# jean-pierreBoth/kmerutils

Measured on AMD Instinct MI355X. Metric: Gbases/sec k-mer+sketch throughput, k=31, 200 sketches/read, higher is better.
Workload: dtype u64; 1 GPU; ont_k31: 746333 ONT-shaped reads (log-normal lengths, 8% errors), 4.38e+09 bases, k=31, ProbMinHash3a m=200 + kmercount 8-bit; workload_name=ont_k31, reads_per_gpu=746333, bases_per_gpu=4379626696, kmers_per_gpu=4357236706, k=31, sketch_size=200, sketch=True, count=True, parallelism=reads sharded x1

## Files before the change

### kmerutils_amd/csrc/kmu_device.h

```cpp
#pragma once

#include <hip/hip_runtime.h>
#include <stdint.h>

#include "../../include/kmu.h"

#define KMU_WAVE 64

namespace kmu {

__device__ __forceinline__ uint32_t code2b(uint32_t c) {
    uint32_t x = (c >> 1) & 3u;
    return x ^ (x >> 1);
}
__device__ __forceinline__ bool is_acgt(uint32_t c) {
    uint32_t u = c & 0xDFu;
    return (u == 'A') | (u == 'C') | (u == 'G') | (u == 'T');
}
__device__ __forceinline__ uint32_t codes4_ascii(uint32_t c) {
    uint32_t x = (c >> 1) & 0x03030303u;
    x ^= (x >> 1) & 0x01010101u;
    return (x * 0x40100401u) >> 24;
}
__device__ __forceinline__ uint32_t diff4_ascii(uint32_t c) {
    const uint32_t u = c & 0xDFDFDFDFu;
    const uint32_t t = (u >> 2) & ~(u >> 1) & 0x01010101u;
    const uint32_t e = 0x40404040u | (u & 0x06060606u) | (t << 4) | (t ^ 0x01010101u);
    return u ^ e;
}
__device__ __forceinline__ uint32_t nonzero4(uint32_t d) {
    const uint32_t nz = (((d & 0x7F7F7F7Fu) + 0x7F7F7F7Fu) | d) & 0x80808080u;
    return (((nz >> 7) * 0x01020408u) >> 24) & 0xFu;
}
__device__ __forceinline__ uint32_t pack16_ascii(uint4 v, uint32_t &bad) {
    const uint32_t out = (codes4_ascii(v.x) << 24) | (codes4_ascii(v.y) << 16) | (codes4_ascii(v.z) << 8) | codes4_ascii(v.w);
    const uint32_t d0 = diff4_ascii(v.x), d1 = diff4_ascii(v.y), d2 = diff4_ascii(v.z), d3 = diff4_ascii(v.w);
    bad = 0;
    if (d0 | d1 | d2 | d3) bad = nonzero4(d0) | (nonzero4(d1) << 4) | (nonzero4(d2) << 8) | (nonzero4(d3) << 12);
    return out;
}
__device__ __forceinline__ uint32_t code_aa(uint32_t c) {
    const uint32_t i = c - 'A';
    const uint64_t t = i < 12u ? 0x52408398a418801ull : i < 24u ? 0x52609460f6818bull : 0x15ull;
    const uint32_t f = i < 12u ? i : i < 24u ? i - 12u : (i - 24u) & 1u;
    return i < 26u ? (uint32_t) (t >> (5u * f)) & 31u : 0u;
}

__device__ __forceinline__ uint64_t revcomp_val(uint64_t val, int k) {
    uint64_t rc = ~val;
    rc = __brevll(rc);
    rc = ((rc & 0x5555555555555555ull) << 1) | ((rc & 0xAAAAAAAAAAAAAAAAull) >> 1);
    return rc >> (64 - 2 * k);
}

struct StepWin {
    uint64_t hi, rlo, kmask;
    uint32_t w2, rhi;
    int sh;
};
__device__ __forceinline__ uint32_t revcomp16(uint32_t w) {
    const uint32_t r = __brev(~w);
    return ((r & 0x55555555u) << 1) | ((r >> 1) & 0x55555555u);
}
__device__ __forceinline__ StepWin step_win(uint32_t w0, uint32_t w1, uint32_t w2, int k) {
    StepWin s;
    s.hi = ((uint64_t) w0 << 32) | w1;
    s.w2 = w2;
    s.rlo = ((uint64_t) revcomp16(w1) << 32) | revcomp16(w0);
    s.rhi = revcomp16(w2);
    s.sh = 64 - 2 * k;
    s.kmask = ~0ull >> (64 - 2 * k);
    return s;
}
__device__ __forceinline__ void step_val_rc(const StepWin &s, uint32_t j, uint64_t &val, uint64_t &rc) {
    val = ((s.hi << (2 * j)) | (((uint64_t) s.w2 << (2 * j)) >> 32)) >> s.sh;
    rc = (j ? (s.rlo >> (2 * j)) | ((uint64_t) s.rhi << (64 - 2 * j)) : s.rlo) & s.kmask;
}
__device__ __forceinline__ uint64_t step_canonical(const StepWin &s, uint32_t j) {
    uint64_t val, rc;
    step_val_rc(s, j, val, rc);
    return rc < val ? rc : val;
}

__device__ __forceinline__ uint32_t int32_hash(uint32_t key) {
    key = ~key + (key << 15);
    key = key ^ (key >> 12);
    key = key + (key << 2);
    key = key ^ (key >> 4);
    key = key * 2057u;
    key = key ^ (key >> 16);
    return key;
}
__device__ __forceinline__ uint64_t int64_hash(uint64_t key) {
    key = ~key + (key << 21);
    key = key ^ (key >> 24);
    key = (key + (key << 3)) + (key << 8);
    key = key ^ (key >> 14);
    key = (key + (key << 2)) + (key << 4);
    key = key ^ (key >> 28);
    key = key + (key << 31);
    return key;
}

__device__ __forceinline__ uint64_t rotl64(uint64_t x, unsigned r) {
    r &= 63u;
    return (x << r) | (x >> ((64u - r) & 63u));
}

__device__ __forceinline__ uint64_t nt_seed(uint32_t code) {
    const uint64_t s[4] = {0x3c8bfbb395c60474ull, 0x3193c18562a02b4cull, 0x20323ed082572324ull,
                           0x295549f54be24456ull};
    return s[code & 3u];
}
__device__ __forceinline__ uint64_t nt8b_fwd(uint32_t code) {
    return code == 0 ? 0x3c8bfbb395c60474ull : (code == 1 ? 0x3193c18562a02b4cull : 0ull);
}
__device__ __forceinline__ uint64_t nt8b_rev(uint32_t code) {
    return code == 0 ? 0x295549f54be24456ull : (code == 1 ? 0x20323ed082572324ull : 0ull);
}
template <bool TABLE8B>
__device__ __forceinline__ uint64_t nthash_canonical(uint64_t val, int k) {
    uint64_t f = 0, r = 0;
    for (int i = 0; i < k; i++) {
        uint32_t b = (uint32_t) (val >> (2 * (k - 1 - i))) & 3u;
        if (TABLE8B) {
            f ^= rotl64(nt8b_fwd(b), (unsigned) (k - i - 1));
            r ^= rotl64(nt8b_rev(b), (unsigned) i);
        } else {
            f ^= rotl64(nt_seed(b), (unsigned) (k - i - 1));
// ... 128 lines not shown
        1.0 / 1124000727777607680000.0};
    double acc = inv_fact[22];
    for (int i = 21; i >= 1; i--) acc = acc * x + inv_fact[i];
    return acc * x;
}

struct Exp01 {
    double lambda, c1, c2, c3;
};
__device__ __forceinline__ double exp01_sample(const Exp01 &e, Xoshiro &rng) {
    double x = e.c1 * rng.unif01();
    if (x < 1.0) return x;
    for (;;) {
        x = rng.unif01();
        if (x < e.c2) return x;
        double y = 0.5 * rng.unif01();
        if (y > 1.0 - x) {
            x = 1.0 - x;
            y = 1.0 - y;
        }
        if (x <= e.c3 * (1.0 - y)) return x;
        if (e.c1 * y <= 1.0 - x) return x;
        if (y * e.c1 * e.lambda <= expm1_small(e.lambda * (1.0 - x))) return x;
    }
}

__device__ __forceinline__ uint32_t bottomk_row_len(const uint64_t *r, uint32_t m) {
    uint32_t n = 0;
    while (n < m && r[n] != 0xFFFFFFFFFFFFFFFFull) n++;
    return n;
}
__device__ __forceinline__ void minhash_walk(const uint64_t *r1, uint32_t n1, const uint64_t *r2, uint32_t n2, uint32_t *out) {
    uint32_t i = 0, j = 0, common = 0, total = 0;
    while (i < n1 && j < n2) {
        const uint64_t x = r1[i], y = r2[j];
        if (x < y) i++;
        else if (y < x) j++;
        else { i++; j++; common++; }
        total++;
        if (total >= n1) break;
    }
    if (total < n1) {
        if (i < n1) total += n1 - i;
        if (j < n1) total += n1 - j;
        if (total > n1) total = n1;
    }
    out[0] = common;
    out[1] = total;
    out[2] = i;
}

__device__ __forceinline__ int lane_id() { return (int) (threadIdx.x & 63u); }
__device__ __forceinline__ void lds_barrier() { asm volatile("s_waitcnt lgkmcnt(0)\n\ts_barrier" ::: "memory"); }
__device__ __forceinline__ uint32_t wave_incl_scan_u32(uint32_t v) {
    v += (uint32_t) __builtin_amdgcn_update_dpp(0, (int) v, 0x111, 0xf, 0xf, false);
    v += (uint32_t) __builtin_amdgcn_update_dpp(0, (int) v, 0x112, 0xf, 0xf, false);
    v += (uint32_t) __builtin_amdgcn_update_dpp(0, (int) v, 0x114, 0xf, 0xf, false);
    v += (uint32_t) __builtin_amdgcn_update_dpp(0, (int) v, 0x118, 0xf, 0xf, false);
    v += (uint32_t) __builtin_amdgcn_update_dpp(0, (int) v, 0x142, 0xa, 0xf, false);
    v += (uint32_t) __builtin_amdgcn_update_dpp(0, (int) v, 0x143, 0xc, 0xf, false);
    return v;
}
__device__ __forceinline__ uint32_t shfl_down_u32(uint32_t v, int d) { return (uint32_t) __shfl_down((int) v, d, 64); }
__device__ __forceinline__ uint32_t bcast_u32(uint32_t v, int src) { return (uint32_t) __shfl((int) v, src, 64); }
__device__ __forceinline__ uint32_t readlane_u32(uint32_t v, uint32_t l) { return (uint32_t) __builtin_amdgcn_readlane((int) v, (int) l); }
__device__ __forceinline__ uint32_t wave_max_u32(uint32_t v) {
    auto mx = [](uint32_t a, uint32_t b) { return a > b ? a : b; };
    v = mx(v, (uint32_t) __builtin_amdgcn_update_dpp(0, (int) v, 0x111, 0xf, 0xf, false));
    v = mx(v, (uint32_t) __builtin_amdgcn_update_dpp(0, (int) v, 0x112, 0xf, 0xf, false));
    v = mx(v, (uint32_t) __builtin_amdgcn_update_dpp(0, (int) v, 0x114, 0xf, 0xf, false));
    v = mx(v, (uint32_t) __builtin_amdgcn_update_dpp(0, (int) v, 0x118, 0xf, 0xf, false));
    v = mx(v, (uint32_t) __builtin_amdgcn_update_dpp(0, (int) v, 0x142, 0xa, 0xf, false));
    v = mx(v, (uint32_t) __builtin_amdgcn_update_dpp(0, (int) v, 0x143, 0xc, 0xf, false));
    return (uint32_t) __builtin_amdgcn_readlane((int) v, 63);
}
__device__ __forceinline__ uint64_t wave_max_u64(uint64_t v) {
#pragma unroll
    for (int d = 32; d >= 1; d >>= 1) {
        uint64_t o = ((uint64_t) (uint32_t) __shfl_xor((int) (v >> 32), d, 64) << 32) |
                     (uint32_t) __shfl_xor((int) (uint32_t) v, d, 64);
        v = o > v ? o : v;
    }
    return v;
}
template <int CTRL, int ROWS> __device__ __forceinline__ uint64_t dpp_u64(uint64_t v) {
    return ((uint64_t) (uint32_t) __builtin_amdgcn_update_dpp(0, (int) (v >> 32), CTRL, ROWS, 0xf, false) << 32) |
           (uint32_t) __builtin_amdgcn_update_dpp(0, (int) (uint32_t) v, CTRL, ROWS, 0xf, false);
}
__device__ __forceinline__ uint64_t wave_max_u64_dpp(uint64_t v) {
    auto mx = [](uint64_t a, uint64_t b) { return a > b ? a : b; };
    v = mx(v, dpp_u64<0x111, 0xf>(v));
    v = mx(v, dpp_u64<0x112, 0xf>(v));
    v = mx(v, dpp_u64<0x114, 0xf>(v));
    v = mx(v, dpp_u64<0x118, 0xf>(v));
    v = mx(v, dpp_u64<0x142, 0xa>(v));
    v = mx(v, dpp_u64<0x143, 0xc>(v));
    return ((uint64_t) readlane_u32((uint32_t) (v >> 32), 63) << 32) | readlane_u32((uint32_t) v, 63);
}
__device__ __forceinline__ uint32_t wave_min_u32(uint32_t v) { return ~wave_max_u32(~v); }
__device__ __forceinline__ uint32_t wave_sum_u32(uint32_t v) {
    for (int o = 32; o >= 1; o >>= 1) v += (uint32_t) __shfl_xor((int) v, o, 64);
    return v;
}
__device__ __forceinline__ uint64_t wave_sum_u64(uint64_t v) {
    for (int o = 32; o >= 1; o >>= 1)
        v += ((uint64_t) (uint32_t) __shfl_xor((int) (v >> 32), o, 64) << 32) | (uint32_t) __shfl_xor((int) (uint32_t) v, o, 64);
// ... 90 lines not shown
```

### kmerutils_amd/csrc/kmu_pmh_long.hip

```cpp
#include "kmu_pmh_steps.h"
#include "kmu_sketch_host.hpp"

namespace kmu {

template <typename T>
__device__ __forceinline__ T ld_scr(const T *p) { return __hip_atomic_load(p, __ATOMIC_RELAXED, __HIP_MEMORY_SCOPE_AGENT); }
template <typename T>
__device__ __forceinline__ void st_scr(T *p, T v) { __hip_atomic_store(p, v, __ATOMIC_RELAXED, __HIP_MEMORY_SCOPE_AGENT); }

__global__ void __launch_bounds__(1024, 4) k_multiset_long(SketchArgs a) {
    constexpr int UQ_THREADS = 1024;
    constexpr uint32_t UQ_BM_BITS = UQ2_BM, UQ_COLL = UQ2_COLL;
    typedef UqShape<UQ_THREADS, UQ_BM_BITS, UQ_COLL> SH;
    constexpr uint32_t UQ_KEYS = SH::KEYS, UQ_BM_WORDS = SH::BM_WORDS, UQ_BUCKETS = SH::BUCKETS, UQ_TILE = SH::TILE;
    constexpr uint32_t TILE_WORDS = UQ_KEYS / 16;
    static_assert((UQ_BM_WORDS / 4) % (uint32_t) UQ_THREADS == 0, "whole 16-byte stores per thread wipe a bitmap");
    static_assert(UQ_COLL % UQ_THREADS == 0 && UQ_COLL / UQ_THREADS <= 4, "collected keys per thread");
    static_assert(TILE_WORDS + 2 <= UQ_TILE, "a tile's words and the two behind them fit the staged words");
    static_assert(UQ_KEYS + UQ_COLL + UQ_COLL / 2 <= DEF_SEG, "a segment holds a sub-list, its collected keys and their weights");
    static_assert(PMH_LONG_TP < UQ_KEYS, "a sub-list of the expected size fits the registers");
    extern __shared__ __attribute__((aligned(16))) uint8_t smem[];
    uint32_t *bmA = reinterpret_cast<uint32_t *>(smem);
    uint32_t *bmB = bmA + UQ_BM_WORDS;
    uint64_t *ck = reinterpret_cast<uint64_t *>(bmB + UQ_BM_WORDS);
    uint64_t *dk = ck + UQ_COLL;
    uint32_t *dw = reinterpret_cast<uint32_t *>(dk + UQ_COLL);
    uint32_t *bst = dw + UQ_COLL;
    uint32_t *words = bst + UQ_BUCKETS + 1;
    uint32_t *wtot = words + UQ_TILE;
    uint32_t *misc = wtot + UQ_THREADS / 64;
    constexpr uint32_t RAW_OFF = ((8u * UQ_BM_WORDS + 20u * UQ_COLL + 4u * (UQ_BUCKETS + 1u + UQ_TILE + (uint32_t) UQ_THREADS / 64u) + 64u) + 15u) & ~15u;
    static_assert(RAW_OFF + 8u * DEF_PARTS <= SH::LDS, "the sub-lists' counters lie inside the shape's LDS");
    uint32_t *pcnt = reinterpret_cast<uint32_t *>(smem + RAW_OFF);
    uint32_t *ccnt = pcnt + DEF_PARTS;
    const KmerCfg cfg = a.cfg;
    const int k = cfg.k, tid = threadIdx.x, lane = lane_id(), wave = tid >> 6;
    uint64_t *seg0 = a.def_keys + (uint64_t) blockIdx.x * DEF_CAP;
    for (uint32_t i = tid; i < UQ_BUCKETS + 1; i += UQ_THREADS) bst[i] = 0;
    auto take = [&]() -> uint32_t {
        if (misc[8] == misc[9]) {
            if (!misc[11]) misc[10] = atomicAdd(a.queue, (uint32_t) QCHUNK);
            misc[8] = misc[10];
            misc[9] = misc[10] + QCHUNK;
            misc[11] = 0;
        }
        const uint32_t v = misc[8]++;
        if (misc[8] == misc[9] && !misc[11]) { misc[10] = atomicAdd(a.queue, (uint32_t) QCHUNK); misc[11] = 1; }
        return v;
    };
    if (tid == 0) {
        misc[8] = misc[9] = misc[10] = misc[11] = 0;
        misc[4] = take();
    }
    __syncthreads();
    const uint64_t off_first = uniform_u64(a.offsets[0]);
    const uint64_t total = a.total_bytes ? a.total_bytes : uniform_u64(a.offsets[a.n_seq]);
    auto seq_of = [&](uint32_t q) -> uint32_t { return a.read_list ? a.read_list[q] : q; };
    uint32_t r = uniform_u32(misc[4]);
    uint32_t rs = r < a.n_queue ? uniform_u32(seq_of(r)) : 0u;
    SeqView sv;
    sv.base = a.bases; sv.packed = 0; sv.total = total; sv.begin = 0; sv.len = 0;
    if (r < a.n_queue) { sv.begin = uniform_u64(a.offsets[rs]); sv.len = uniform_u64(a.offsets[rs + 1]) - sv.begin; }
    auto place_of = [&](int q) -> uint32_t { return 4u * ((uint32_t) tid + (uint32_t) UQ_THREADS * (uint32_t) (q >> 2)) + (uint32_t) (q & 3); };
    auto bm_index = [&](uint64_t key) -> uint32_t {
        return (((uint32_t) key ^ (uint32_t) (key >> 32)) * 0x85EBCA6Bu) >> (32 - UQ_BM_BITS);
    };
    while (r < a.n_queue) {
        if (tid == 0) {
            misc[5] = take();
            misc[0] = 0;
        }
        if (tid < (int) DEF_PARTS) pcnt[tid] = 0;
        const uint32_t L = sv.len >= 0x80000000ull ? 0xFFFFFFFFu : (uint32_t) sv.len;
        const uint32_t nk = L >= (uint32_t) k ? L - (uint32_t) k + 1u : 0u;
        const uint32_t lead = seq_lead(sv), wfirst = lead >> 4, l0 = lead - 16u * wfirst;
        const uint32_t span = uniform_u32(nk + l0);
        const uint32_t P = uniform_u32(pmh_long_parts(nk));
        const bool mine = nk >= 1u && L != 0xFFFFFFFFu && span > UQ_KEYS && P <= DEF_PARTS;
        uint32_t bad = 0;
        lds_barrier();
        const uint32_t r_next = uniform_u32(misc[5]);
        const bool has_next = r_next < a.n_queue;
        const uint32_t rs_n = has_next ? seq_of(r_next) : 0u;
        const uint64_t n_o0 = has_next ? a.offsets[rs_n] : 0ull, n_o1 = has_next ? a.offsets[rs_n + 1] : 0ull;
        bool over = false;
        uint32_t n_u = 0, n_ct = 0;
        if (mine) {
            const uint32_t nw_all = (uint32_t) ((L - 1 + lead) >> 4) + 2;
            auto scan_phase = [&](auto fast_tag) __attribute__((always_inline)) {
                constexpr bool FAST = decltype(fast_tag)::value;
                for (uint32_t t0 = 0; t0 < span; t0 += UQ_KEYS) {
                    const uint32_t w0 = t0 >> 4;
                    const uint32_t nwt = nw_all - w0 < TILE_WORDS + 2 ? nw_all - w0 : TILE_WORDS + 2;
                    for (uint32_t t = tid; t < nwt; t += UQ_THREADS) {
                        uint32_t b;
                        words[t] = load_code_word(sv, (uint64_t) wfirst + w0 + t, b);
                        bad |= b;
                    }
                    lds_barrier();
                    const uint32_t span_t = span - t0;
#pragma unroll
                    for (int q0 = 0; q0 < UQ_KREG; q0 += 4) {
                        if (!(4u * (uint32_t) UQ_THREADS * (uint32_t) (q0 >> 2) < span_t)) continue;
                        const uint32_t wi = ((uint32_t) tid >> 2) + (uint32_t) (UQ_THREADS / 4) * (uint32_t) (q0 >> 2);
                        const StepWin sw = step_win(words[wi], words[wi + 1], words[wi + 2], k);
                        uint64_t key[4];
                        uint32_t part[4], at[4];
#pragma unroll
                        for (int u = 0; u < 4; u++) {
                            key[u] = 0;
                            part[u] = 0xFFFFFFFFu;
                            if (t0 + place_of(q0 + u) - l0 < nk) {
                                uint64_t val, rc;
                                step_val_rc(sw, 4u * ((uint32_t) tid & 3u) + (uint32_t) u, val, rc);
                                key[u] = FAST ? int64_hash(rc < val ? rc : val) : apply_fhash(cfg, val, rc);
                                part[u] = pmh_long_part_of(key[u], P);
                            }
                        }
#pragma unroll
                        for (int u = 0; u < 4; u++) {
                            at[u] = 0xFFFFFFFFu;
                            if (part[u] != 0xFFFFFFFFu) at[u] = atomicAdd(&pcnt[part[u]], 1u);
                        }
#pragma unroll
                        for (int u = 0; u < 4; u++)
                            if (at[u] < UQ_KEYS) st_scr(&seg0[(uint64_t) part[u] * DEF_SEG + at[u]], key[u]);
                    }
                    lds_barrier();
                }
            };
            if (cfg.fhash == KMU_FHASH_CANON_INVHASH && cfg.kmer_type == KMU_KMER64BIT) scan_phase(std::true_type{});
            else scan_phase(std::false_type{});
            __syncthreads();
            const uint64_t lb = sv.begin - off_first;
            for (uint32_t p = 0; p < P && !over; p++) {
                const uint32_t n_p = uniform_u32(pcnt[p]);
                if (n_p > UQ_KEYS) { over = true; break; }
                uint64_t *seg = seg0 + (uint64_t) p * DEF_SEG;
                uint4 *za = reinterpret_cast<uint4 *>(bmA), *zb = reinterpret_cast<uint4 *>(bmB);
#pragma unroll
                for (uint32_t z = 0; z < UQ_BM_WORDS / 4 / (uint32_t) UQ_THREADS; z++) {
                    za[tid + z * UQ_THREADS] = make_uint4(0u, 0u, 0u, 0u);
                    zb[tid + z * UQ_THREADS] = make_uint4(0u, 0u, 0u, 0u);
                }
                if (tid == 0) misc[1] = 0;
                lds_barrier();
                auto group_used = [&](int q0) -> bool { return 4u * (uint32_t) UQ_THREADS * (uint32_t) (q0 >> 2) < n_p; };
                uint64_t rk[UQ_KREG];
#pragma unroll
                for (int q0 = 0; q0 < UQ_KREG; q0 += 4) {
                    if (!group_used(q0)) {
#pragma unroll
                        for (int u = 0; u < 4; u++) rk[q0 + u] = __builtin_nondeterministic_value(rk[q0 + u]);
                        continue;
                    }
                    uint32_t bit[4], rbw[4], rbb[4];
#pragma unroll
                    for (int u = 0; u < 4; u++) {
                        const uint32_t e = (uint32_t) (q0 + u) * UQ_THREADS + (uint32_t) tid;
                        rk[q0 + u] = 0;
                        if (e < n_p) rk[q0 + u] = ld_scr(&seg[e]);
                    }
#pragma unroll
                    for (int u = 0; u < 4; u++) {
                        const uint32_t e = (uint32_t) (q0 + u) * UQ_THREADS + (uint32_t) tid;
                        const uint32_t bi = bm_index(rk[q0 + u]);
                        rbw[u] = e < n_p ? bi >> 5 : (uint32_t) tid;
                        rbb[u] = e < n_p ? 1u << (bi & 31u) : 0u;
                    }
#pragma unroll
                    for (int u = 0; u < 4; u++) bit[u] = atomicOr(&bmA[rbw[u]], rbb[u]);
#pragma unroll
                    for (int u = 0; u < 4; u++) bit[u] &= rbb[u];
#pragma unroll
                    for (int u = 0; u < 4; u++)
                        if (bit[u]) atomicOr(&bmB[rbw[u]], bit[u]);
                }
                lds_barrier();
#pragma unroll
                for (int q0 = 0; q0 < UQ_KREG; q0 += 4) {
                    if (!group_used(q0)) continue;
                    bool uq[4], co[4];
                    uint64_t um[4], cm[4];
                    uint32_t ut = 0, ct = 0, bw[4];
#pragma unroll
                    for (int u = 0; u < 4; u++) bw[u] = bmB[bm_index(rk[q0 + u]) >> 5];
#pragma unroll
                    for (int u = 0; u < 4; u++) {
                        const bool have = (uint32_t) (q0 + u) * UQ_THREADS + (uint32_t) tid < n_p;
                        co[u] = have && (bw[u] & (1u << (bm_index(rk[q0 + u]) & 31u))) != 0u;
                        uq[u] = have && !co[u];
                    }
#pragma unroll
                    for (int u = 0; u < 4; u++) {
                        um[u] = __ballot(uq[u]);
                        cm[u] = __ballot(co[u]);
                        ut += (uint32_t) __popcll(um[u]);
                        ct += (uint32_t) __popcll(cm[u]);
                    }
                    uint32_t ub = 0, cb = 0;
                    if (lane == 0) {
                        if (ut) ub = atomicAdd(&misc[0], ut);
                        if (ct) cb = atomicAdd(&misc[1], ct);
                    }
                    ub = bcast_u32(ub, 0);
                    cb = bcast_u32(cb, 0);
#pragma unroll
                    for (int u = 0; u < 4; u++) {
                        const uint64_t below = (1ull << lane) - 1ull;
                        if (uq[u]) {
                            const uint64_t at = lb + ub + (uint32_t) __popcll(um[u] & below);
                            a.lst_keys[at] = rk[q0 + u];
                        }
                        if (co[u]) {
                            const uint32_t at = cb + (uint32_t) __popcll(cm[u] & below);
                            if (at < UQ_COLL) ck[at] = rk[q0 + u];
                        }
                        ub += (uint32_t) __popcll(um[u]);
                        cb += (uint32_t) __popcll(cm[u]);
                    }
                }
                lds_barrier();
                const uint32_t n_c = uniform_u32(misc[1]);
                if (n_c > UQ_COLL) { over = true; break; }
                if (tid == 0) ccnt[p] = n_c;
                if (n_c) {
                    uint64_t key[UQ_COLL / UQ_THREADS];
                    uint32_t rb[UQ_COLL / UQ_THREADS];
#pragma unroll
                    for (int j = 0; j < (int) (UQ_COLL / UQ_THREADS); j++) {
                        const uint32_t i = (uint32_t) j * UQ_THREADS + tid;
                        rb[j] = 0xFFFFFFFFu;
                        key[j] = 0;
                        if (i < n_c) {
                            key[j] = ck[i];
                            const uint32_t b = mix32(key[j]) / (0x80000000u / (UQ_BUCKETS / 2));
                            rb[j] = (b << 16) | atomicAdd(&bst[b], 1u);
                        }
                    }
                    lds_barrier();
                    {
                        const uint32_t c0 = bst[2 * tid], c1 = bst[2 * tid + 1];
                        const uint32_t incl = wave_incl_scan_u32(c0 + c1);
                        if (lane == 63) wtot[wave] = incl;
                        lds_barrier();
                        uint32_t pre = incl - (c0 + c1);
#pragma unroll
                        for (int w = 0; w < UQ_THREADS / 64; w++) pre += w < wave ? wtot[w] : 0u;
                        bst[2 * tid] = pre;
                        bst[2 * tid + 1] = pre + c0;
                    }
                    lds_barrier();
#pragma unroll
                    for (int j = 0; j < (int) (UQ_COLL / UQ_THREADS); j++)
                        if (rb[j] != 0xFFFFFFFFu) {
                            const uint32_t pos = bst[rb[j] >> 16] + (rb[j] & 0xFFFFu);
                            rb[j] = (rb[j] & 0xFFFF0000u) | pos;
                            dk[pos] = key[j];
                            dw[pos] = 1u;
                        }
                    lds_barrier();
#pragma unroll
                    for (int j = 0; j < (int) (UQ_COLL / UQ_THREADS); j++)
                        if (rb[j] != 0xFFFFFFFFu) {
                            const uint32_t pos = rb[j] & 0xFFFFu;
                            for (uint32_t t = bst[rb[j] >> 16]; t < pos; t++)
                                if (dk[t] == key[j]) {
                                    dw[pos] = 0u;
                                    atomicAdd(&dw[t], 1u);
                                    break;
                                }
                        }
                    lds_barrier();
                    uint32_t *seg_w = reinterpret_cast<uint32_t *>(seg + UQ_KEYS + UQ_COLL);
                    for (uint32_t i = tid; i < n_c; i += UQ_THREADS) {
                        st_scr(&seg[UQ_KEYS + i], dk[i]);
                        st_scr(&seg_w[i], dw[i]);
                    }
                    bst[2 * tid] = 0;
                    bst[2 * tid + 1] = 0;
                }
                lds_barrier();
            }
            __syncthreads();
            if (!over) {
                n_u = uniform_u32(misc[0]);
                for (uint32_t p = 0; p < P; p++) {
                    const uint32_t n_c = uniform_u32(ccnt[p]);
                    const uint64_t *seg = seg0 + (uint64_t) p * DEF_SEG;
                    const uint32_t *seg_w = reinterpret_cast<const uint32_t *>(seg + UQ_KEYS + UQ_COLL);
                    for (uint32_t i = tid; i < n_c; i += UQ_THREADS) {
                        a.lst_keys[lb + n_u + n_ct + i] = ld_scr(&seg[UQ_KEYS + i]);
                        a.lst_w[lb + n_u + n_ct + i] = ld_scr(&seg_w[i]);
                    }
                    n_ct += n_c;
                }
            }
        }
        if (tid == 0) {
            if (mine && !over) { a.lst_n[rs] = n_u + n_ct; a.lst_nu[rs] = n_u; }
            else if (nk != 0) {
                a.lst_n[rs] = 0u;
                a.lst_nu[rs] = 0u;
                a.redo_list[atomicAdd(a.queue + 56, 1u)] = rs;
            }
        }
        if (bad) atomicOr(a.err, DERR_NON_ACGT);
        r = r_next;
        rs = uniform_u32(rs_n);
        if (has_next) {
            sv.begin = uniform_u64(n_o0);
            sv.len = uniform_u64(n_o1) - sv.begin;
        }
        lds_barrier();
    }
}

}
```

### kmerutils_amd/csrc/kmu_pmh_uq.hip

```cpp
#include "kmu_pmh_steps.h"

namespace kmu {

__device__ __forceinline__ void vm_wait_lds_loads() {
    __builtin_amdgcn_s_waitcnt(0x0F70);
    asm volatile("" ::: "memory");
}

template <int UQ_THREADS, uint32_t UQ_BM_BITS, uint32_t UQ_COLL, int MINW>
__global__ void __launch_bounds__(UQ_THREADS, MINW) k_multiset_uq(SketchArgs a) {
    typedef UqShape<UQ_THREADS, UQ_BM_BITS, UQ_COLL> SH;
    constexpr uint32_t UQ_KEYS = SH::KEYS, UQ_BM_WORDS = SH::BM_WORDS, UQ_BUCKETS = SH::BUCKETS, UQ_TILE = SH::TILE;
    static_assert((UQ_BM_WORDS / 4) % (uint32_t) UQ_THREADS == 0, "whole 16-byte stores per thread wipe a bitmap");
    static_assert(UQ_COLL % UQ_THREADS == 0 && UQ_COLL / UQ_THREADS <= 4, "collected keys per thread");
    static_assert((uint32_t) UQ_THREADS <= UQ_BM_WORDS, "every thread has a word of bitmap A of its own");
    extern __shared__ __attribute__((aligned(16))) uint8_t smem[];
    uint32_t *bmA = reinterpret_cast<uint32_t *>(smem);
    uint32_t *bmB = bmA + UQ_BM_WORDS;
    uint64_t *ck = reinterpret_cast<uint64_t *>(bmB + UQ_BM_WORDS);
    uint64_t *dk = ck + UQ_COLL;
    uint32_t *dw = reinterpret_cast<uint32_t *>(dk + UQ_COLL);
    uint32_t *bst = dw + UQ_COLL;
    uint32_t *words = bst + UQ_BUCKETS + 1;
    uint32_t *wtot = words + UQ_TILE;
    uint32_t *misc = wtot + UQ_THREADS / 64;
    constexpr uint32_t RAW_OFF = ((8u * UQ_BM_WORDS + 20u * UQ_COLL + 4u * (UQ_BUCKETS + 1u + UQ_TILE + (uint32_t) UQ_THREADS / 64u) + 64u) + 15u) & ~15u;
    uint8_t *rawp = smem + RAW_OFF;
    const KmerCfg cfg = a.cfg;
    const int k = cfg.k, tid = threadIdx.x, lane = lane_id(), wave = tid >> 6;
    for (uint32_t i = tid; i < UQ_BUCKETS + 1; i += UQ_THREADS) bst[i] = 0;
    auto take = [&]() -> uint32_t {
        if (misc[8] == misc[9]) {
            if (!misc[11]) misc[10] = atomicAdd(a.queue, (uint32_t) QCHUNK);
            misc[8] = misc[10];
            misc[9] = misc[10] + QCHUNK;
            misc[11] = 0;
        }
        const uint32_t v = misc[8]++;
        if (misc[8] == misc[9] && !misc[11]) { misc[10] = atomicAdd(a.queue, (uint32_t) QCHUNK); misc[11] = 1; }
        return v;
    };
    if (tid == 0) {
        misc[8] = misc[9] = misc[10] = misc[11] = 0;
        misc[4] = take();
        misc[5] = take();
    }
    __syncthreads();
    const uint64_t off_first = uniform_u64(a.offsets[0]);
    const uint64_t total = a.total_bytes ? a.total_bytes : uniform_u64(a.offsets[a.n_seq]);
    auto seq_of = [&](uint32_t q) -> uint32_t { return a.read_list ? a.read_list[q] : q; };
    uint32_t r = uniform_u32(misc[4]);
    uint32_t rs = r < a.n_queue ? uniform_u32(seq_of(r)) : 0u;
    SeqView sv;
    sv.base = a.bases; sv.packed = 0; sv.total = total; sv.begin = 0; sv.len = 0;
    if (r < a.n_queue) { sv.begin = uniform_u64(a.offsets[rs]); sv.len = uniform_u64(a.offsets[rs + 1]) - sv.begin; }
    auto fits = [&](const SeqView &v) -> bool {
        const uint32_t Lv = v.len >= 0x80000000ull ? 0xFFFFFFFFu : (uint32_t) v.len;
        return Lv >= (uint32_t) k && Lv - (uint32_t) k + 1u + seq_lead(v) <= UQ_KEYS;
    };
    static_assert(UQ_KREG % 4 == 0 && UQ_THREADS % 4 == 0, "quarters of words");
    auto place_of = [&](int q) -> uint32_t { return 4u * ((uint32_t) tid + (uint32_t) UQ_THREADS * (uint32_t) (q >> 2)) + (uint32_t) (q & 3); };
    uint32_t r_next = uniform_u32(misc[5]);
    uint32_t rs_next = r_next < a.n_queue ? uniform_u32(seq_of(r_next)) : 0u;
    SeqView nv = sv;
    bool nv_mine = false;
    if (r_next < a.n_queue) {
        nv.begin = uniform_u64(a.offsets[rs_next]);
        nv.len = uniform_u64(a.offsets[rs_next + 1]) - nv.begin;
        nv_mine = fits(nv);
    }
    __syncthreads();
    uint32_t pf_bad = 0;
    bool pf_valid = false;
    auto n_words = [&](const SeqView &v) -> uint32_t {
        const uint32_t Lv = (uint32_t) v.len, ld = seq_lead(v);
        return (uint32_t) ((Lv - 1 + ld) >> 4) + 2;
    };
    while (r < a.n_queue) {
        if (tid == 0) {
            misc[5] = take();
            misc[0] = 0;
            misc[1] = 0;
        }
        const uint32_t L = sv.len >= 0x80000000ull ? 0xFFFFFFFFu : (uint32_t) sv.len;
        const uint32_t nk = L >= (uint32_t) k ? L - (uint32_t) k + 1u : 0u;
        const bool mine = nk >= 1u && nk + seq_lead(sv) <= UQ_KEYS;
        uint32_t bad = 0;
        if (L == 0 && tid == 0) atomicOr(a.err, DERR_EMPTY_SEQ);
        if (nk == 0) bad |= wave_validate_seq(sv, wave, UQ_THREADS / 64, false);
        const uint32_t lead = seq_lead(sv), wfirst = lead >> 4;
        if (mine) {
            const uint32_t nw = n_words(sv);
            if (pf_valid) bad |= pf_bad;
            else {
                for (uint32_t t = tid; t < nw; t += UQ_THREADS) {
                    uint32_t b;
                    words[t] = load_code_word(sv, (uint64_t) wfirst + t, b);
                    bad |= b;
                }
            }
            uint4 *za = reinterpret_cast<uint4 *>(bmA), *zb = reinterpret_cast<uint4 *>(bmB);
#pragma unroll
            for (uint32_t z = 0; z < UQ_BM_WORDS / 4 / (uint32_t) UQ_THREADS; z++) {
                za[tid + z * UQ_THREADS] = make_uint4(0u, 0u, 0u, 0u);
                zb[tid + z * UQ_THREADS] = make_uint4(0u, 0u, 0u, 0u);
            }
        }
        lds_barrier();
        const uint32_t r_nn = uniform_u32(misc[5]);
        const bool has_nn = r_nn < a.n_queue;
        const uint32_t rs_nn = has_nn ? seq_of(r_nn) : 0u;
        const uint64_t nn_o0 = has_nn ? a.offsets[rs_nn] : 0ull, nn_o1 = has_nn ? a.offsets[rs_nn + 1] : 0ull;
        uint32_t nwn = 0, wfn = 0;
        if (nv_mine) {
            nwn = n_words(nv);
            wfn = seq_lead(nv) >> 4;
#pragma unroll
            for (int u = 0; u < 3; u++) {
                const uint32_t tw = (uint32_t) tid + (uint32_t) u * UQ_THREADS;
                if (tw < nwn && chunk_is_plain(nv, (uint64_t) wfn + tw))
                    chunk16_to_lds_uncounted(nv.base + (nv.begin & ~15ull) + 16 * ((uint64_t) wfn + tw),
                                             lds_addr(smem) + RAW_OFF + (uint32_t) (wave + u * (UQ_THREADS / 64)) * 1024u);
            }
        }
        uint64_t rk[UQ_KREG];
        auto bm_index = [&](uint64_t key) -> uint32_t {
            return (((uint32_t) key ^ (uint32_t) (key >> 32)) * 0x85EBCA6Bu) >> (32 - UQ_BM_BITS);
        };
        const uint32_t span = uniform_u32(nk + (lead - 16u * wfirst));
        auto group_used = [&](int q0) -> bool { return 4u * (uint32_t) UQ_THREADS * (uint32_t) (q0 >> 2) < span; };
        bool over = false;
        if (mine) {
            const uint32_t l0 = lead - 16u * wfirst;
            auto key_phase = [&](auto fast_tag) __attribute__((always_inline)) {
                constexpr bool FAST = decltype(fast_tag)::value;
#pragma unroll
                for (int q0 = 0; q0 < UQ_KREG; q0 += 4) {
                    if (!group_used(q0)) {
#pragma unroll
                        for (int u = 0; u < 4; u++) rk[q0 + u] = __builtin_nondeterministic_value(rk[q0 + u]);
                        continue;
                    }
                    uint32_t bit[4], rbw[4], rbb[4];
                    const uint32_t wi = ((uint32_t) tid >> 2) + (uint32_t) (UQ_THREADS / 4) * (uint32_t) (q0 >> 2);
                    const StepWin sw = step_win(words[wi], words[wi + 1], words[wi + 2], k);
#pragma unroll
                    for (int u = 0; u < 4; u++) {
                        const int q = q0 + u;
                        rbw[u] = (uint32_t) tid;
                        rbb[u] = 0;
                        rk[q] = 0;
                        if (place_of(q) - l0 < nk) {
                            uint64_t val, rc;
                            step_val_rc(sw, 4u * ((uint32_t) tid & 3u) + (uint32_t) u, val, rc);
                            const uint64_t key = FAST ? int64_hash(rc < val ? rc : val) : apply_fhash(cfg, val, rc);
                            rk[q] = key;
                            const uint32_t bi = bm_index(key);
                            rbw[u] = bi >> 5;
                            rbb[u] = 1u << (bi & 31u);
                        }
                    }
#pragma unroll
                    for (int u = 0; u < 4; u++) bit[u] = atomicOr(&bmA[rbw[u]], rbb[u]);
#pragma unroll
                    for (int u = 0; u < 4; u++) bit[u] &= rbb[u];
#pragma unroll
                    for (int u = 0; u < 4; u++)
                        if (bit[u]) atomicOr(&bmB[rbw[u]], bit[u]);
                }
            };
            if (cfg.fhash == KMU_FHASH_CANON_INVHASH && cfg.kmer_type == KMU_KMER64BIT) key_phase(std::true_type{});
            else key_phase(std::false_type{});
            lds_barrier();
        }
        if (nv_mine) {
            vm_wait_lds_loads();
            pf_bad = 0;
#pragma unroll
            for (int u = 0; u < 3; u++) {
                const uint32_t tw = (uint32_t) tid + (uint32_t) u * UQ_THREADS;
                uint32_t b = 0;
                if (tw < nwn)
                    words[tw] = chunk_is_plain(nv, (uint64_t) wfn + tw)
                                    ? code_word_from_chunk(nv, (uint64_t) wfn + tw, *reinterpret_cast<const u32x4 *>(rawp + (size_t) tw * 16), b)
                                    : load_code_word(nv, (uint64_t) wfn + tw, b);
                pf_bad |= b;
            }
        }
        const uint64_t lb = sv.begin - off_first;
        if (mine) {
#pragma unroll
            for (int q0 = 0; q0 < UQ_KREG; q0 += 4) {
                if (!group_used(q0)) continue;
                bool uq[4], co[4];
                uint64_t um[4], cm[4];
                uint32_t ut = 0, ct = 0, bw[4];
#pragma unroll
                for (int u = 0; u < 4; u++) bw[u] = bmB[bm_index(rk[q0 + u]) >> 5];
#pragma unroll
                for (int u = 0; u < 4; u++) {
                    const int q = q0 + u;
                    const bool have = place_of(q) - (lead - 16u * wfirst) < nk;
                    co[u] = have && (bw[u] & (1u << (bm_index(rk[q]) & 31u))) != 0u;
                    uq[u] = have && !co[u];
                }
#pragma unroll
                for (int u = 0; u < 4; u++) {
                    um[u] = __ballot(uq[u]);
                    cm[u] = __ballot(co[u]);
                    ut += (uint32_t) __popcll(um[u]);
                    ct += (uint32_t) __popcll(cm[u]);
                }
                uint32_t ub = 0, cb = 0;
                if (lane == 0) {
                    if (ut) ub = atomicAdd(&misc[0], ut);
                    if (ct) cb = atomicAdd(&misc[1], ct);
                }
                ub = bcast_u32(ub, 0);
                cb = bcast_u32(cb, 0);
#pragma unroll
                for (int u = 0; u < 4; u++) {
                    const uint64_t below = (1ull << lane) - 1ull;
                    if (uq[u]) {
                        const uint64_t at = lb + ub + (uint32_t) __popcll(um[u] & below);
                        a.lst_keys[at] = rk[q0 + u];
                    }
                    if (co[u]) {
                        const uint32_t at = cb + (uint32_t) __popcll(cm[u] & below);
                        if (at < UQ_COLL) ck[at] = rk[q0 + u];
                    }
                    ub += (uint32_t) __popcll(um[u]);
                    cb += (uint32_t) __popcll(cm[u]);
                }
            }
            lds_barrier();
            const uint32_t n_u = uniform_u32(misc[0]), n_c = uniform_u32(misc[1]);
            over = n_c > UQ_COLL;
            if (!over && n_c) {
                uint64_t key[UQ_COLL / UQ_THREADS];
                uint32_t rb[UQ_COLL / UQ_THREADS];
#pragma unroll
                for (int j = 0; j < (int) (UQ_COLL / UQ_THREADS); j++) {
                    const uint32_t i = (uint32_t) j * UQ_THREADS + tid;
                    rb[j] = 0xFFFFFFFFu;
                    key[j] = 0;
                    if (i < n_c) {
                        key[j] = ck[i];
                        const uint32_t b = mix32(key[j]) / (0x80000000u / (UQ_BUCKETS / 2));
                        rb[j] = (b << 16) | atomicAdd(&bst[b], 1u);
                    }
                }
                lds_barrier();
                {
                    const uint32_t c0 = bst[2 * tid], c1 = bst[2 * tid + 1];
                    const uint32_t incl = wave_incl_scan_u32(c0 + c1);
                    if (lane == 63) wtot[wave] = incl;
                    lds_barrier();
                    uint32_t pre = incl - (c0 + c1);
#pragma unroll
                    for (int w = 0; w < UQ_THREADS / 64; w++) pre += w < wave ? wtot[w] : 0u;
                    bst[2 * tid] = pre;
                    bst[2 * tid + 1] = pre + c0;
                }
                lds_barrier();
#pragma unroll
                for (int j = 0; j < (int) (UQ_COLL / UQ_THREADS); j++)
                    if (rb[j] != 0xFFFFFFFFu) {
                        const uint32_t pos = bst[rb[j] >> 16] + (rb[j] & 0xFFFFu);
                        rb[j] = (rb[j] & 0xFFFF0000u) | pos;
                        dk[pos] = key[j];
                        dw[pos] = 1u;
                    }
                lds_barrier();
#pragma unroll
                for (int j = 0; j < (int) (UQ_COLL / UQ_THREADS); j++)
                    if (rb[j] != 0xFFFFFFFFu) {
                        const uint32_t pos = rb[j] & 0xFFFFu;
                        for (uint32_t t = bst[rb[j] >> 16]; t < pos; t++)
                            if (dk[t] == key[j]) {
                                dw[pos] = 0u;
                                atomicAdd(&dw[t], 1u);
                                break;
                            }
                    }
                lds_barrier();
                for (uint32_t i = tid; i < n_c; i += UQ_THREADS) {
                    a.lst_keys[lb + n_u + i] = dk[i];
                    a.lst_w[lb + n_u + i] = dw[i];
                }
                bst[2 * tid] = 0;
                bst[2 * tid + 1] = 0;
            }
            if (tid == 0 && !over) { a.lst_n[rs] = n_u + n_c; a.lst_nu[rs] = n_u; }
        }
        if (tid == 0) {
            if (nk == 0) a.lst_n[rs] = 0u;
            else if (!mine || over) {
                a.lst_n[rs] = 0u;
                a.redo_list[atomicAdd(a.queue + 56, 1u)] = rs;
            }
        }
        if (bad) atomicOr(a.err, DERR_NON_ACGT);
        pf_valid = nv_mine;
        r = r_next;
        rs = rs_next;
        sv = nv;
        r_next = r_nn;
        rs_next = uniform_u32(rs_nn);
        nv_mine = false;
        if (has_nn) {
            nv.begin = uniform_u64(nn_o0);
            nv.len = uniform_u64(nn_o1) - nv.begin;
            nv_mine = fits(nv);
        }
        lds_barrier();
    }
}

#define KMU_X_INST(...) template __global__ void __VA_ARGS__(SketchArgs);
KMU_PMH_UQ_FORMS(KMU_X_INST)
#undef KMU_X_INST

}
```

### kmerutils_amd/csrc/kmu_sketch_kernels.h

```cpp
#pragma once

#include "kmu_ctx.hpp"
#include "kmu_device.h"

namespace kmu {

struct SketchArgs {
    const uint8_t *bases;
    const uint64_t *offsets;
    const uint64_t *packed_offsets;
    const uint64_t *block_rows;
    uint32_t n_seq;
    int packed;
    uint64_t total_bytes;
    KmerCfg cfg;
    int m;
    int hasher;
    int rand08;
    int sig_bytes;
    uint32_t block_size;
    uint32_t cap;
    uint32_t part_target;
    double inv_part_target;
    uint32_t tile_shift;
    uint64_t *scr_keys;
    uint32_t *scr_info;
    uint32_t *scr_w;
    uint32_t skip_longer;
    uint64_t *def_keys;
    int bk_shift;
    uint32_t bk_mask;
    uint32_t *tau_redo;
    double tau_num;
    uint32_t *counts_out;
    const void *hashed;
    int hashed_bytes;
    uint64_t *part_h;
    uint64_t *part_k;
    uint64_t *lst_keys;
    uint32_t *lst_w;
    uint32_t *lst_n;
    uint32_t *lst_nu;
    uint32_t *queue2;
    uint32_t *pts_long;
    uint32_t pts_long_t;
    uint32_t *redo_list;
    const uint32_t *read_list;
    uint32_t n_queue;
    uint32_t tile_words;
    uint32_t idx_thresh;
    uint64_t idx_zone;
    uint32_t tau_min_n;
    Exp01 e01;
    void *sig_out;
    uint32_t *queue;
    uint32_t *err;
};

enum { M_READ = 0, M_NSCR = 1, M_NEXT = 2, M_DEF = 3, M_QMAX = 4 , M_FLAGS = 6 , M_WORDS = 8 };
static constexpr uint32_t DEF_CAP = 1u << 20;
static constexpr uint32_t DEF_PARTS = 32;
static constexpr uint32_t DEF_SEG = DEF_CAP / DEF_PARTS;
static constexpr uint32_t LONG_SEQ_KMERS = 1u << 18;
static constexpr int BUCKET_BITS = 12;
static constexpr uint32_t NBUCKETS = 1u << BUCKET_BITS;
static constexpr int QCHUNK = 4;
static constexpr int KREG = 10;
static constexpr uint32_t WINV_LUT = 256;
static constexpr size_t PTS_WAVE_WORDS = 2 + 128 + 64 + 256;
static constexpr double PTS_TAU_C = 4.6;
static constexpr int UQ_KREG = 20;
static constexpr uint32_t UQ1_BM = 17, UQ1_COLL = 1024, UQ2_BM = 18, UQ2_COLL = 2048;
template <int UQ_THREADS, uint32_t UQ_BM_BITS, uint32_t UQ_COLL>
struct UqShape {
    static constexpr uint32_t KEYS = (uint32_t) UQ_THREADS * UQ_KREG;
    static constexpr uint32_t BM_WORDS = (1u << UQ_BM_BITS) / 32;
    static constexpr uint32_t BUCKETS = 2u * UQ_THREADS;
    static constexpr uint32_t TILE = (KEYS + 32 + 15) / 16 + 3;
    static constexpr uint32_t RAW_WAVES = (TILE + 63) / 64;
    static constexpr size_t LDS = (size_t) BM_WORDS * 8 + (size_t) UQ_COLL * 20 + ((size_t) BUCKETS + 1 + TILE + UQ_THREADS / 64 + 8 + 8) * 4 + 64 +
                                  (size_t) RAW_WAVES * 1024 + 16;
};
static constexpr uint32_t SHORT_KEYS = 256, SHORT_SLOTS = 512, SHORT_WORDS = 24;
static constexpr size_t SHORT_WAVE_BYTES = (size_t) SHORT_SLOTS * 12 + SHORT_WORDS * 4;
static constexpr uint32_t SMALLK_WORDS = 32768;
static constexpr uint32_t SMALLK_TILE = 1024;

template <bool AA, bool BOTTOMK, bool EMIT = false, bool PLAIN = false>
__global__ void __launch_bounds__(1024) k_sketch_pmh3a(SketchArgs a);
__global__ void k_pts_long_list(const uint32_t *lst_n, uint32_t n_seq, uint32_t thr, uint32_t *out);
template <bool SIG32>
__global__ void __launch_bounds__(256) k_pmh_points(SketchArgs a);
template <int UQ_THREADS, uint32_t UQ_BM_BITS, uint32_t UQ_COLL, int MINW>
__global__ void __launch_bounds__(UQ_THREADS, MINW) k_multiset_uq(SketchArgs a);
__global__ void __launch_bounds__(1024, 4) k_multiset_long(SketchArgs a);
__global__ void k_multiset_short(SketchArgs a);
template <bool SIG32>
__global__ void __launch_bounds__(256) k_pmh_points_short(SketchArgs a);
template <bool EMIT>
__global__ void __launch_bounds__(1024) k_sketch_smallk(SketchArgs a);
__global__ void k_pmh_reduce(const uint64_t *part_h, const uint64_t *part_k, uint64_t n_parts, int m, uint64_t stride, int sig_bytes, void *sig_out,
                             uint64_t *part_out);
__global__ void k_max_len(const uint64_t *offsets, uint32_t n_seq, uint64_t *out);
__global__ void k_nk_scan(const uint64_t *offsets, uint32_t n_seq, int k, uint64_t *koff, uint32_t *err);
__global__ void k_seq_hashes_compact(const uint8_t *bases, const uint64_t *offsets, const uint64_t *packed_offsets, uint32_t n_seq, int packed,
                                     uint64_t total, KmerCfg cfg, const uint64_t *koff, uint64_t *out, uint32_t *err, int spread);
__global__ void k_widen_u32(const uint32_t *in, uint64_t n, uint64_t *out);

#define KMU_PMH_GENERAL_FORMS(X)                                                                                                    \
    X(k_sketch_pmh3a<false, false>) X(k_sketch_pmh3a<false, false, true>) X(k_sketch_pmh3a<true, true>) X(k_sketch_pmh3a<true, false>) \
// ... 13 lines not shown
```

Measured before the change: 54.31 Gbases/s.

## Reload cold kernel args lazily, hide constants from hoisting, deepen read lookahead

Result: faster. 55.09 Gbases/s, median of 6 (+1.4%).

```diff
diff --git a/kmerutils_amd/csrc/kmu_device.h b/kmerutils_amd/csrc/kmu_device.h
--- a/kmerutils_amd/csrc/kmu_device.h
+++ b/kmerutils_amd/csrc/kmu_device.h
@@ -75,6 +75,10 @@
 __device__ __forceinline__ void step_val_rc(const StepWin &s, uint32_t j, uint64_t &val, uint64_t &rc) {
     val = ((s.hi << (2 * j)) | (((uint64_t) s.w2 << (2 * j)) >> 32)) >> s.sh;
     rc = (j ? (s.rlo >> (2 * j)) | ((uint64_t) s.rhi << (64 - 2 * j)) : s.rlo) & s.kmask;
+}
+__device__ __forceinline__ void step_val_rc_lane(const StepWin &s, uint32_t j, uint64_t &val, uint64_t &rc) {
+    val = ((s.hi << (2 * j)) | (((uint64_t) s.w2 << (2 * j)) >> 32)) >> s.sh;
+    rc = ((s.rlo >> (2 * j)) | (((uint64_t) s.rhi << 32) << (32 - 2 * j))) & s.kmask;
 }
 __device__ __forceinline__ uint64_t step_canonical(const StepWin &s, uint32_t j) {
     uint64_t val, rc;
@@ -309,6 +313,25 @@
 
 __device__ __forceinline__ int lane_id() { return (int) (threadIdx.x & 63u); }
 __device__ __forceinline__ void lds_barrier() { asm volatile("s_waitcnt lgkmcnt(0)\n\ts_barrier" ::: "memory"); }
+template <typename T>
+__device__ __forceinline__ T kernarg_at(uint32_t byte_off) {
+    const __attribute__((address_space(4))) uint8_t *p =
+        (const __attribute__((address_space(4))) uint8_t *) __builtin_amdgcn_kernarg_segment_ptr();
+    asm volatile("" : "+s"(p));
+    return *reinterpret_cast<const __attribute__((address_space(4))) T *>(p + byte_off);
+}
+__device__ __forceinline__ uint32_t opaque_u32(uint32_t v) {
+    asm volatile("" : "+s"(v));
+    return v;
+}
+__device__ __forceinline__ uint32_t opaque_lane_u32(uint32_t v) {
+    asm volatile("" : "+v"(v));
+    return v;
+}
+template <typename T>
+__device__ __forceinline__ T *lane_ptr(T *p, uint32_t byte_off) {
+    return reinterpret_cast<T *>(reinterpret_cast<uint8_t *>(p) + byte_off);
+}
 __device__ __forceinline__ uint32_t wave_incl_scan_u32(uint32_t v) {
     v += (uint32_t) __builtin_amdgcn_update_dpp(0, (int) v, 0x111, 0xf, 0xf, false);
     v += (uint32_t) __builtin_amdgcn_update_dpp(0, (int) v, 0x112, 0xf, 0xf, false);
diff --git a/kmerutils_amd/csrc/kmu_pmh_long.hip b/kmerutils_amd/csrc/kmu_pmh_long.hip
--- a/kmerutils_amd/csrc/kmu_pmh_long.hip
+++ b/kmerutils_amd/csrc/kmu_pmh_long.hip
@@ -39,13 +39,13 @@
     for (uint32_t i = tid; i < UQ_BUCKETS + 1; i += UQ_THREADS) bst[i] = 0;
     auto take = [&]() -> uint32_t {
         if (misc[8] == misc[9]) {
-            if (!misc[11]) misc[10] = atomicAdd(a.queue, (uint32_t) QCHUNK);
+            if (!misc[11]) misc[10] = atomicAdd(KMU_COLD_ARG(queue), (uint32_t) QCHUNK);
             misc[8] = misc[10];
             misc[9] = misc[10] + QCHUNK;
             misc[11] = 0;
         }
         const uint32_t v = misc[8]++;
-        if (misc[8] == misc[9] && !misc[11]) { misc[10] = atomicAdd(a.queue, (uint32_t) QCHUNK); misc[11] = 1; }
+        if (misc[8] == misc[9] && !misc[11]) { misc[10] = atomicAdd(KMU_COLD_ARG(queue), (uint32_t) QCHUNK); misc[11] = 1; }
         return v;
     };
     if (tid == 0) {
@@ -55,7 +55,10 @@
     __syncthreads();
     const uint64_t off_first = uniform_u64(a.offsets[0]);
     const uint64_t total = a.total_bytes ? a.total_bytes : uniform_u64(a.offsets[a.n_seq]);
-    auto seq_of = [&](uint32_t q) -> uint32_t { return a.read_list ? a.read_list[q] : q; };
+    auto seq_of = [&](uint32_t q) -> uint32_t {
+        const uint32_t *rl = KMU_COLD_ARG(read_list);
+        return rl ? rl[q] : q;
+    };
     uint32_t r = uniform_u32(misc[4]);
     uint32_t rs = r < a.n_queue ? uniform_u32(seq_of(r)) : 0u;
     SeqView sv;
@@ -99,11 +102,12 @@
                     }
                     lds_barrier();
                     const uint32_t span_t = span - t0;
+                    const int kq = (int) opaque_u32((uint32_t) k);
 #pragma unroll
                     for (int q0 = 0; q0 < UQ_KREG; q0 += 4) {
                         if (!(4u * (uint32_t) UQ_THREADS * (uint32_t) (q0 >> 2) < span_t)) continue;
                         const uint32_t wi = ((uint32_t) tid >> 2) + (uint32_t) (UQ_THREADS / 4) * (uint32_t) (q0 >> 2);
-                        const StepWin sw = step_win(words[wi], words[wi + 1], words[wi + 2], k);
+                        const StepWin sw = step_win(words[wi], words[wi + 1], words[wi + 2], kq);
                         uint64_t key[4];
                         uint32_t part[4], at[4];
 #pragma unroll
@@ -112,7 +116,7 @@
                             part[u] = 0xFFFFFFFFu;
                             if (t0 + place_of(q0 + u) - l0 < nk) {
                                 uint64_t val, rc;
-                                step_val_rc(sw, 4u * ((uint32_t) tid & 3u) + (uint32_t) u, val, rc);
+                                step_val_rc_lane(sw, 4u * ((uint32_t) tid & 3u) + (uint32_t) u, val, rc);
                                 key[u] = FAST ? int64_hash(rc < val ? rc : val) : apply_fhash(cfg, val, rc);
                                 part[u] = pmh_long_part_of(key[u], P);
                             }
@@ -199,9 +203,10 @@
                         ct += (uint32_t) __popcll(cm[u]);
                     }
                     uint32_t ub = 0, cb = 0;
-                    if (lane == 0) {
-                        if (ut) ub = atomicAdd(&misc[0], ut);
-                        if (ct) cb = atomicAdd(&misc[1], ct);
+                    const uint32_t ln = opaque_lane_u32((uint32_t) lane), z0 = opaque_lane_u32(0u);
+                    if (ln == 0) {
+                        if (ut) ub = atomicAdd(lane_ptr(misc, z0), ut);
+                        if (ct) cb = atomicAdd(lane_ptr(misc + 1, z0), ct);
                     }
                     ub = bcast_u32(ub, 0);
                     cb = bcast_u32(cb, 0);
@@ -285,27 +290,28 @@
             __syncthreads();
             if (!over) {
                 n_u = uniform_u32(misc[0]);
+                uint32_t *lst_w = KMU_COLD_ARG(lst_w);
                 for (uint32_t p = 0; p < P; p++) {
                     const uint32_t n_c = uniform_u32(ccnt[p]);
                     const uint64_t *seg = seg0 + (uint64_t) p * DEF_SEG;
                     const uint32_t *seg_w = reinterpret_cast<const uint32_t *>(seg + UQ_KEYS + UQ_COLL);
                     for (uint32_t i = tid; i < n_c; i += UQ_THREADS) {
                         a.lst_keys[lb + n_u + n_ct + i] = ld_scr(&seg[UQ_KEYS + i]);
-                        a.lst_w[lb + n_u + n_ct + i] = ld_scr(&seg_w[i]);
+                        lst_w[lb + n_u + n_ct + i] = ld_scr(&seg_w[i]);
                     }
                     n_ct += n_c;
                 }
             }
         }
         if (tid == 0) {
-            if (mine && !over) { a.lst_n[rs] = n_u + n_ct; a.lst_nu[rs] = n_u; }
+            if (mine && !over) { KMU_COLD_ARG(lst_n)[rs] = n_u + n_ct; KMU_COLD_ARG(lst_nu)[rs] = n_u; }
             else if (nk != 0) {
-                a.lst_n[rs] = 0u;
-                a.lst_nu[rs] = 0u;
-                a.redo_list[atomicAdd(a.queue + 56, 1u)] = rs;
+                KMU_COLD_ARG(lst_n)[rs] = 0u;
+                KMU_COLD_ARG(lst_nu)[rs] = 0u;
+                KMU_COLD_ARG(redo_list)[atomicAdd(KMU_COLD_ARG(queue) + 56, 1u)] = rs;
             }
         }
-        if (bad) atomicOr(a.err, DERR_NON_ACGT);
+        if (bad) atomicOr(KMU_COLD_ARG(err), DERR_NON_ACGT);
         r = r_next;
         rs = uniform_u32(rs_n);
         if (has_next) {
diff --git a/kmerutils_amd/csrc/kmu_pmh_uq.hip b/kmerutils_amd/csrc/kmu_pmh_uq.hip
--- a/kmerutils_amd/csrc/kmu_pmh_uq.hip
+++ b/kmerutils_amd/csrc/kmu_pmh_uq.hip
@@ -31,24 +31,28 @@
     for (uint32_t i = tid; i < UQ_BUCKETS + 1; i += UQ_THREADS) bst[i] = 0;
     auto take = [&]() -> uint32_t {
         if (misc[8] == misc[9]) {
-            if (!misc[11]) misc[10] = atomicAdd(a.queue, (uint32_t) QCHUNK);
+            if (!misc[11]) misc[10] = atomicAdd(KMU_COLD_ARG(queue), (uint32_t) QCHUNK);
             misc[8] = misc[10];
             misc[9] = misc[10] + QCHUNK;
             misc[11] = 0;
         }
         const uint32_t v = misc[8]++;
-        if (misc[8] == misc[9] && !misc[11]) { misc[10] = atomicAdd(a.queue, (uint32_t) QCHUNK); misc[11] = 1; }
+        if (misc[8] == misc[9] && !misc[11]) { misc[10] = atomicAdd(KMU_COLD_ARG(queue), (uint32_t) QCHUNK); misc[11] = 1; }
         return v;
     };
     if (tid == 0) {
         misc[8] = misc[9] = misc[10] = misc[11] = 0;
         misc[4] = take();
         misc[5] = take();
+        misc[6] = take();
     }
     __syncthreads();
     const uint64_t off_first = uniform_u64(a.offsets[0]);
     const uint64_t total = a.total_bytes ? a.total_bytes : uniform_u64(a.offsets[a.n_seq]);
-    auto seq_of = [&](uint32_t q) -> uint32_t { return a.read_list ? a.read_list[q] : q; };
+    auto seq_of = [&](uint32_t q) -> uint32_t {
+        const uint32_t *rl = KMU_COLD_ARG(read_list);
+        return rl ? rl[q] : q;
+    };
     uint32_t r = uniform_u32(misc[4]);
     uint32_t rs = r < a.n_queue ? uniform_u32(seq_of(r)) : 0u;
     SeqView sv;
@@ -69,6 +73,8 @@
         nv.len = uniform_u64(a.offsets[rs_next + 1]) - nv.begin;
         nv_mine = fits(nv);
     }
+    uint32_t r_nn = uniform_u32(misc[6]);
+    uint32_t rs_nn = r_nn < a.n_queue ? uniform_u32(seq_of(r_nn)) : 0u;
     __syncthreads();
     uint32_t pf_bad = 0;
     bool pf_valid = false;
@@ -78,7 +84,7 @@
     };
     while (r < a.n_queue) {
         if (tid == 0) {
-            misc[5] = take();
+            misc[6] = take();
             misc[0] = 0;
             misc[1] = 0;
         }
@@ -86,7 +92,7 @@
         const uint32_t nk = L >= (uint32_t) k ? L - (uint32_t) k + 1u : 0u;
         const bool mine = nk >= 1u && nk + seq_lead(sv) <= UQ_KEYS;
         uint32_t bad = 0;
-        if (L == 0 && tid == 0) atomicOr(a.err, DERR_EMPTY_SEQ);
+        if (L == 0 && tid == 0) atomicOr(KMU_COLD_ARG(err), DERR_EMPTY_SEQ);
         if (nk == 0) bad |= wave_validate_seq(sv, wave, UQ_THREADS / 64, false);
         const uint32_t lead = seq_lead(sv), wfirst = lead >> 4;
         if (mine) {
@@ -107,9 +113,9 @@
             }
         }
         lds_barrier();
-        const uint32_t r_nn = uniform_u32(misc[5]);
         const bool has_nn = r_nn < a.n_queue;
-        const uint32_t rs_nn = has_nn ? seq_of(r_nn) : 0u;
+        const uint32_t r_n3 = uniform_u32(misc[6]);
+        const uint32_t rs_n3 = r_n3 < a.n_queue ? seq_of(r_n3) : 0u;
         const uint64_t nn_o0 = has_nn ? a.offsets[rs_nn] : 0ull, nn_o1 = has_nn ? a.offsets[rs_nn + 1] : 0ull;
         uint32_t nwn = 0, wfn = 0;
         if (nv_mine) {
@@ -134,6 +140,7 @@
             const uint32_t l0 = lead - 16u * wfirst;
             auto key_phase = [&](auto fast_tag) __attribute__((always_inline)) {
                 constexpr bool FAST = decltype(fast_tag)::value;
+                const int kq = (int) opaque_u32((uint32_t) k);
 #pragma unroll
                 for (int q0 = 0; q0 < UQ_KREG; q0 += 4) {
                     if (!group_used(q0)) {
@@ -143,7 +150,7 @@
                     }
                     uint32_t bit[4], rbw[4], rbb[4];
                     const uint32_t wi = ((uint32_t) tid >> 2) + (uint32_t) (UQ_THREADS / 4) * (uint32_t) (q0 >> 2);
-                    const StepWin sw = step_win(words[wi], words[wi + 1], words[wi + 2], k);
+                    const StepWin sw = step_win(words[wi], words[wi + 1], words[wi + 2], kq);
 #pragma unroll
                     for (int u = 0; u < 4; u++) {
                         const int q = q0 + u;
@@ -152,7 +159,7 @@
                         rk[q] = 0;
                         if (place_of(q) - l0 < nk) {
                             uint64_t val, rc;
-                            step_val_rc(sw, 4u * ((uint32_t) tid & 3u) + (uint32_t) u, val, rc);
+                            step_val_rc_lane(sw, 4u * ((uint32_t) tid & 3u) + (uint32_t) u, val, rc);
                             const uint64_t key = FAST ? int64_hash(rc < val ? rc : val) : apply_fhash(cfg, val, rc);
                             rk[q] = key;
                             const uint32_t bi = bm_index(key);
@@ -212,9 +219,10 @@
                     ct += (uint32_t) __popcll(cm[u]);
                 }
                 uint32_t ub = 0, cb = 0;
-                if (lane == 0) {
-                    if (ut) ub = atomicAdd(&misc[0], ut);
-                    if (ct) cb = atomicAdd(&misc[1], ct);
+                const uint32_t ln = opaque_lane_u32((uint32_t) lane), z0 = opaque_lane_u32(0u);
+                if (ln == 0) {
+                    if (ut) ub = atomicAdd(lane_ptr(misc, z0), ut);
+                    if (ct) cb = atomicAdd(lane_ptr(misc + 1, z0), ct);
                 }
                 ub = bcast_u32(ub, 0);
                 cb = bcast_u32(cb, 0);
@@ -284,29 +292,32 @@
                             }
                     }
                 lds_barrier();
+                uint32_t *lst_w = KMU_COLD_ARG(lst_w);
                 for (uint32_t i = tid; i < n_c; i += UQ_THREADS) {
                     a.lst_keys[lb + n_u + i] = dk[i];
-                    a.lst_w[lb + n_u + i] = dw[i];
+                    lst_w[lb + n_u + i] = dw[i];
                 }
                 bst[2 * tid] = 0;
                 bst[2 * tid + 1] = 0;
             }
-            if (tid == 0 && !over) { a.lst_n[rs] = n_u + n_c; a.lst_nu[rs] = n_u; }
+            if (tid == 0 && !over) { KMU_COLD_ARG(lst_n)[rs] = n_u + n_c; KMU_COLD_ARG(lst_nu)[rs] = n_u; }
         }
         if (tid == 0) {
-            if (nk == 0) a.lst_n[rs] = 0u;
+            if (nk == 0) KMU_COLD_ARG(lst_n)[rs] = 0u;
             else if (!mine || over) {
-                a.lst_n[rs] = 0u;
-                a.redo_list[atomicAdd(a.queue + 56, 1u)] = rs;
-            }
-        }
-        if (bad) atomicOr(a.err, DERR_NON_ACGT);
+                KMU_COLD_ARG(lst_n)[rs] = 0u;
+                KMU_COLD_ARG(redo_list)[atomicAdd(KMU_COLD_ARG(queue) + 56, 1u)] = rs;
+            }
+        }
+        if (bad) atomicOr(KMU_COLD_ARG(err), DERR_NON_ACGT);
         pf_valid = nv_mine;
         r = r_next;
         rs = rs_next;
         sv = nv;
         r_next = r_nn;
-        rs_next = uniform_u32(rs_nn);
+        rs_next = rs_nn;
+        r_nn = r_n3;
+        rs_nn = uniform_u32(rs_n3);
         nv_mine = false;
         if (has_nn) {
             nv.begin = uniform_u64(nn_o0);
diff --git a/kmerutils_amd/csrc/kmu_sketch_kernels.h b/kmerutils_amd/csrc/kmu_sketch_kernels.h
--- a/kmerutils_amd/csrc/kmu_sketch_kernels.h
+++ b/kmerutils_amd/csrc/kmu_sketch_kernels.h
@@ -56,6 +56,7 @@
     uint32_t *queue;
     uint32_t *err;
 };
+#define KMU_COLD_ARG(f) kernarg_at<decltype(SketchArgs::f)>((uint32_t) offsetof(SketchArgs, f))
 
 enum { M_READ = 0, M_NSCR = 1, M_NEXT = 2, M_DEF = 3, M_QMAX = 4 , M_FLAGS = 6 , M_WORDS = 8 };
 static constexpr uint32_t DEF_CAP = 1u << 20;
```
